# visionml/pytracking

Measured on AMD Instinct MI355X. Metric: frames/sec DiMP-50 online track (288x288, 5 SD iters), higher is better.
Workload: dtype f32; 1 GPU; BASELINE configs[1]: DiMP-50 single sequence per GPU; per frame classify(1x512x18x18) + arg-max + memory insert + DiMPSteepestDescentGN(5 it) over n=50x512x18x18, K=4; sequences_per_gpu=1, parallelism=1 independent sequences

## Files before the change

pytracking_amd/csrc/fast_passes.hip:

```cpp
#include "common.h"
#include "pt_internal.h"
#include "sd_common.h"
#include <type_traits>

#ifndef PT_ADJ_WAVES
#define PT_ADJ_WAVES 8
#endif
#ifndef PT_ADJ_UMAX
#define PT_ADJ_UMAX (128 / PT_ADJ_WAVES)
#endif
#ifndef PT_ADJ_UMAX_WIDE
#define PT_ADJ_UMAX_WIDE (192 / PT_ADJ_WAVES)
#endif
#ifndef PT_C2_CD
#define PT_C2_CD 2
#endif
#ifndef PT_C2_MINW
#define PT_C2_MINW 6
#endif
#ifndef PT_ADJ_PD
#define PT_ADJ_PD 3
#endif
#define PT_ADJ_AHEAD 5

#ifdef PT_STAMPS
static unsigned long long* g_pt_stamps = nullptr;
extern "C" void pt_debug_set_stamps(void* p) { g_pt_stamps = (unsigned long long*)p; }
#define PT_STAMP_ARG unsigned long long* stamps;
#define PT_STAMP_SET(a) (a).stamps = g_pt_stamps
#define PT_STAMP(a, k)                                                                                       \
    do {                                                                                                     \
        if ((a).stamps && (threadIdx.x & 63) == 0) {                                                         \
            unsigned long long* sp_ = (a).stamps + ((long)blockIdx.x * 16 + (threadIdx.x >> 6)) * 16;        \
            sp_[(k) < 8 ? (k) : (k) + 1] = (unsigned long long)wall_clock64();                               \
            if ((k) == 0) sp_[8] = (unsigned long long)__builtin_amdgcn_s_getreg((31 << 11) | 4) | (1ull << 32); \
        }                                                                                                    \
    } while (0)
#else
#define PT_STAMP_ARG
#define PT_STAMP_SET(a)
#define PT_STAMP(a, k)
#endif
#if defined(PT_STAMPS) && PT_STAMPS == 2
#define PT_STAMP_A(a, k)
#define PT_STAMP_A_ARRIVED(a, k, v)
#define PT_STAMP_B(a, k) PT_STAMP(a, k)
#else
#define PT_STAMP_A(a, k) PT_STAMP(a, k)
#ifdef PT_STAMPS
#define PT_STAMP_A_ARRIVED(a, k, v)                                                                          \
    do {                                                                                                     \
        asm volatile("" ::"v"(v));                                                                           \
        PT_STAMP(a, k);                                                                                      \
    } while (0)
#else
#define PT_STAMP_A_ARRIVED(a, k, v)
#endif
#define PT_STAMP_B(a, k)
#endif

PtFast pt_fast_plan(int n, int C, int H, int W, int KH, int KW, int OH, int OW) {
    PtFast p;
    p.ok = 0;
    p.n = n; p.C = C; p.H = H; p.W = W; p.KH = KH; p.KW = KW; p.OH = OH; p.OW = OW;
    p.HW = H * W; p.KK = KH * KW; p.OO = OH * OW;
    if ((p.HW % 4) != 0 || W < 4 || p.KK > 16) return p;
    if (C != 64 && C != 128 && C != 256 && C != 512 && C != 1024) return p;
    if ((long)n * p.HW >= (1L << 20)) return p;
    if ((long)n * C * p.HW * 4 >= (1L << 31)) return p;
    p.Q = p.HW / 4;
    p.TF = p.Q / 16;
    p.rem = p.Q % 16;
    p.left = (p.rem > 0 && p.rem <= 4) ? 1 : 0;
    p.tiles = p.TF + ((p.rem > 0 && !p.left) ? 1 : 0);
    if (p.TF < 1 || p.tiles > 16) return p;
    p.nh = 2 * p.tiles <= 10 ? 2 : 1;
    p.CX = C / 8;
    p.KSC = 8;
    if (C == 64) { p.CX = C; p.KSC = 1; }
    p.spw = 1;
    if (p.nh == 2 && p.KSC == 8 && p.CX / 4 <= 16 && (n % 2) == 0 && 8 * n > 256) { p.nh = 1; p.spw = 2; }
    p.NK = p.CX / 4 / p.nh;
    if (p.NK > 16) return p;
    p.mix = (p.spw == 2 && p.tiles == 5 && p.KK == 16 && p.NK >= 4) ? 1 : 0;
    p.HWp = 64 * (p.TF + (p.rem > 0 ? 1 : 0)) + 4;
    p.corr_threads = p.mix ? (2 * p.tiles + 2) * 64 : p.spw * p.nh * p.tiles * 64;
    p.corr_lds = ((size_t)p.CX * 16 + (size_t)p.spw * p.nh * p.KK * p.HWp) * sizeof(float);
    p.sa_direct = (KH == 4 && KW == 4 && p.CX * 16 >= 2 * W + 2) ? 1 : 0;
    if (p.sa_direct && p.HWp < p.HW + 2 * W + 2) p.corr_lds += (size_t)(p.HW + 2 * W + 2 - p.HWp) * sizeof(float);
    if (p.corr_lds > 150 * 1024) return p;
    p.CB = C / 16;
    p.bpx = p.CB / 8;
    p.NG = (int)(((long)n * p.HW + 15) / 16);
    p.KSPL = 0;
    p.E = p.OO <= 384 ? 6 : (p.OO <= 576 ? 9 : 16);
    const int umax = p.E == 9 ? PT_ADJ_UMAX_WIDE : PT_ADJ_UMAX;
    for (int ks = 8; ks <= (p.CB < 8 ? 64 : 16); ks *= 2) {
        const int gper = pt_ceil_div(p.NG, ks), U = pt_ceil_div(gper, PT_ADJ_WAVES);
        if (U <= umax) { p.gper = gper; p.U = U; p.KSPL = pt_ceil_div(p.NG, gper); break; }
    }
    if (p.KSPL == 0) return p;
    p.PH = H + KH - 1;
    p.PW = W + KW - 1;
    while ((p.PW % 16) != 8) ++p.PW;
    p.ns_max = (p.gper * 16 + p.HW - 1) / p.HW + 1;
    p.zn = (KH - 1) * p.PW + KW + 4;
    while (((p.ns_max * p.PH * p.PW + p.zn) % 4) != 0) ++p.zn;
    p.adj_lds = ((size_t)p.ns_max * p.PH * p.PW + p.zn + (size_t)5 * 4 * PT_ADJ_WAVES * umax) * sizeof(float);
    if (p.adj_lds > 96 * 1024 || p.OO > 1024) return p;
    if (H > 255 || W > 255 || n > 65535 || p.gper > 65535 || p.PH > 63 || p.PW > 63 || p.zn > 255 || p.ns_max > 63 || KH > 7 || KW > 7)
        return p;
    p.ok = 1;
    return p;
}

__device__ __forceinline__ int fdiv(int v, float inv_d) { return (int)(((float)v + 0.5f) * inv_d); }

struct Corr2Args {
    pt_gcf feat; long stride_n; pt_gcf filt; pt_gf spart;
    int n, C, H, W, KH, KW, OH, OW, CX, TF, rem, tiles, HWp, nh, KSC;
    int sa_direct;
    pt_gcf gpart; int KSPL; pt_gcf w; float reg; float step; pt_gf g_out; pt_gf anum_part;
    int slot; pt_gcf src; pt_gf copy_dst;
    PT_STAMP_ARG
};

__device__ __forceinline__ float corr2_filter_elem(const Corr2Args& a, int KK, int cx0, int e, bool publish, float& gsq) {
    const int cl = e >> 4, tp = e & 15;
    const bool ok = tp < KK;
    const long ge = (long)(cx0 + cl) * KK + (ok ? tp : 0);
    float v;
    if (a.gpart) {
        const long CKK = (long)a.C * KK;
        v = 0.f;
        for (int k = 0; k < a.KSPL; ++k) v += a.gpart[(long)k * CKK + ge];
        v += a.reg * a.w[ge];
        if (ok) {
            gsq += v * v;
            if (publish) a.g_out[ge] = v;
        }
    } else {
        v = a.filt[ge];
    }
    return ok ? v : 0.f;
}

template <int NK, bool LEFT, int FUSE, bool K16, int NH, bool MIX = false>
__global__ __launch_bounds__(1024, (NK <= 8 && NH == 2 ? PT_C2_MINW : 4)) void k_corr2(const float* h_feat, long h_stride, const float* h_filt, const float* h_w, const float* h_src, int h_slot,
                                                                              unsigned h_dims, unsigned h_geo, unsigned h_aux, Corr2Args a_arg) {
    extern __shared__ __attribute__((aligned(16))) float lds[];
    __shared__ float scratch[16];
    PT_STAMP(a_arg, 0);
    constexpr int EPT = 2;
    constexpr int FP = FUSE > 0 ? FUSE : 1;
    const int hC = (int)(h_dims >> 16), HW = (int)(h_dims & 0xffffu);
    const int h_tiles = (int)(h_geo & 31u), h_TF = (int)((h_geo >> 5) & 31u), h_rem = (int)((h_geo >> 10) & 15u);
    const int h_KSPL = (int)((h_geo >> 14) & 63u);
    const bool ksc16 = ((h_geo >> 20) & 1u) != 0, ksc1 = ((h_geo >> 21) & 1u) != 0, pair = ((h_geo >> 22) & 1u) != 0;
    const int wps = NH * h_tiles;
    const int nthreads = MIX ? (2 * h_tiles + 2) * 64 : (pair ? 2 : 1) * wps * 64;
    const int hCX = ksc1 ? hC : (ksc16 ? hC >> 4 : hC >> 3), hHWp = 64 * (h_TF + (h_rem > 0 ? 1 : 0)) + 4;
    const int b = blockIdx.x, xc = b & 7, q = b >> 3;
    const int x = ksc1 ? 0 : (ksc16 ? 2 * xc + (q & 1) : xc), i0 = ksc1 ? b : (ksc16 ? q >> 1 : q);
    const int KK = K16 ? 16 : a_arg.KH * a_arg.KW;
    const int lane = threadIdx.x & 63, wave = __builtin_amdgcn_readfirstlane(threadIdx.x >> 6);
    const int kq = lane >> 4, j = lane & 15;
    const bool half = MIX && wave < 4;
    const int ws = MIX ? (half ? wave >> 1 : (wave - 4 >= h_tiles - 1 ? 1 : 0)) : ((pair && wave >= wps) ? 1 : 0);
    const int wl = wave - ws * wps;
    const int i = pair ? 2 * i0 + ws : i0;
    const int h = MIX ? (half ? wave & 1 : 0) : (wl >= h_tiles ? 1 : 0);
    const int t = MIX ? (half ? 0 : wave - 3 - ws * (h_tiles - 1)) : wl - h * h_tiles;
    const bool lt = LEFT && t == 0 && (!MIX || h == 0);
    const int cx0 = hCX * x;
    const int nsl = hCX * 16;
    float* __restrict__ afilt = lds;
    float* __restrict__ Tl = lds + nsl + (long)(ws * NH + (MIX ? 0 : h)) * KK * hHWp;
    const bool over = h_src != nullptr && i == h_slot;
    const float* __restrict__ fi = over ? h_src : h_feat + (long)i * h_stride;
    const bool publish = FUSE != 0 && i0 == 0;
    const int h_n = (int)(h_geo >> 23);
    float lz_q = 0.f, lz_an = 0.f;

    constexpr bool k16 = K16;
    const int n4 = nsl >> 1;
    const int e4 = min((int)threadIdx.x, n4 - 1);
    f32x2 part4[FP], wv4 = {0, 0};
    float part[EPT][FP], wv[EPT];
    long gev[EPT];
    bool okv[EPT];
    if (k16) {
        const long g4 = ((long)cx0 * 16 >> 1) + e4;
        if (FUSE > 0) {
            const unsigned ckk_b = (unsigned)hC * 16u * 4u;
            const __amdgpu_buffer_rsrc_t rg = pt_rsrc(h_filt, (unsigned)h_KSPL * ckk_b);
#pragma unroll
            for (int k = 0; k < FP; ++k)
                part4[k] = __builtin_bit_cast(f32x2, __builtin_amdgcn_raw_buffer_load_b64(rg, (unsigned)g4 * 8u, (unsigned)min(k, h_KSPL - 1) * ckk_b, 0));
            wv4 = ((const f32x2*)h_w)[g4];
        } else if (FUSE < 0) {
            part4[0] = ((const f32x2*)h_filt)[g4];
            wv4 = ((const f32x2*)h_w)[g4];
            const float* __restrict__ anp = h_w + h_aux;
            lz_an = lane < (ksc16 ? 16 : (ksc1 ? 1 : 8)) ? anp[lane] : 0.f;
            lz_q = lane < h_n ? anp[64 + lane] : 0.f;
        } else {
            part4[0] = ((const f32x2*)h_filt)[g4];
        }
    } else {
#pragma unroll
        for (int q = 0; q < EPT; ++q) {
            const int e = threadIdx.x + q * nthreads;
            const int ec = min(e, nsl - 1);
            const int cl = ec >> 4, tp = ec & 15;
            okv[q] = e < nsl && tp < KK;
            gev[q] = (long)(cx0 + cl) * KK + (tp < KK ? tp : 0);
            if (FUSE > 0) {
                const long CKK = (long)hC * KK;
#pragma unroll
                for (int k = 0; k < FP; ++k) part[q][k] = h_filt[(long)min(k, h_KSPL - 1) * CKK + gev[q]];
                wv[q] = h_w[gev[q]];
            } else {
                part[q][0] = h_filt[gev[q]];
            }
        }
    }

    constexpr int CD = NK < PT_C2_CD ? NK : PT_C2_CD;
    const int cbase = cx0 + 4 * ((MIX ? 0 : h) * NK) + kq;
    const int pos = 64 * t + 4 * j + (half ? 2 * h : 0);
    const bool pv = pos < HW;
    const __amdgpu_buffer_rsrc_t fr = pt_rsrc(fi, (unsigned)hC * HW * 4u);
    const unsigned fo = ((unsigned)cbase * HW + (pv ? pos : 0)) * 4u;
    const int lpos = 64 * h_TF + j;
    const bool lv = lt && j < 4 * h_rem;
    const unsigned lo = lv ? ((unsigned)cbase * HW + lpos) * 4u : 0xFFFFFFF0u - 64u * (unsigned)HW * 4u;
    f32x4 bq[NK];
    float bl[NK];
    auto ldf = [&](int k) {
        if (MIX && half) {
            const f32x2 v = __builtin_bit_cast(f32x2, __builtin_amdgcn_raw_buffer_load_b64(fr, fo + (unsigned)(4 * k) * HW * 4u, 0, 0));
            bq[k] = (f32x4){v[0], v[1], 0.f, 0.f};
        } else {
            bq[k] = pt_bload4(fr, fo + (unsigned)(4 * k) * HW * 4u);
        }
    };
    auto ldq = [&](int k) {
        ldf(k);
        if (lt) bl[k] = pt_bload1(fr, lo + (unsigned)(4 * k) * HW * 4u);
    };
    if (lt) {
#pragma unroll
        for (int k = 0; k < CD; ++k) bl[k] = pt_bload1(fr, lo + (unsigned)(4 * k) * HW * 4u);
    }
#pragma unroll
    for (int k = 0; k < CD; ++k) ldf(k);
    __builtin_amdgcn_sched_barrier(0);
    const Corr2Args a = pt_late_args<Corr2Args>(56);
    PT_STAMP(a, 1);

    float gsq = 0.f;
    if (k16) {
        f32x2 v4;
        if (FUSE > 0) {
            v4 = (f32x2){0, 0};
#pragma unroll
            for (int k = 0; k < FP; ++k)
                if (k < h_KSPL) v4 += part4[k];
            v4 += a.reg * wv4;
            if ((int)threadIdx.x < n4) {
                gsq = v4[0] * v4[0] + v4[1] * v4[1];
                if (publish) ((f32x2*)a.g_out)[((long)cx0 * 16 >> 1) + e4] = v4;
            }
        } else if (FUSE < 0) {
            float qt = 0.f;
            for (int k = lane + 64; k < h_n; k += 64) qt += (h_w + h_aux)[64 + k];
            const float astep = sd_final_astep(lz_q, qt, lz_an, a.step, a.reg);
            v4 = (f32x2){sd_final_apply(part4[0][0], wv4[0], astep), sd_final_apply(part4[0][1], wv4[1], astep)};
            if ((int)threadIdx.x < n4 && publish) ((f32x2*)a.g_out)[((long)cx0 * 16 >> 1) + e4] = v4;
        } else {
            v4 = part4[0];
        }
        if ((int)threadIdx.x < n4) ((f32x2*)afilt)[e4] = v4;
        for (int q4 = threadIdx.x + nthreads; q4 < n4; q4 += nthreads)
            for (int m = 0; m < 2; ++m) afilt[2 * q4 + m] = corr2_filter_elem(a, KK, cx0, 2 * q4 + m, publish, gsq);
    } else {
#pragma unroll
        for (int q = 0; q < EPT; ++q) {
            const int e = threadIdx.x + q * nthreads;
            float v;
            if (FUSE > 0) {
                v = 0.f;
#pragma unroll
                for (int k = 0; k < FP; ++k) v += k < h_KSPL ? part[q][k] : 0.f;
                v += a.reg * wv[q];
                if (okv[q]) {
                    gsq += v * v;
                    if (publish) a.g_out[gev[q]] = v;
                }
            } else {
                v = part[q][0];
            }
            if (e < nsl) afilt[e] = okv[q] ? v : 0.f;
        }
        for (int e = threadIdx.x + EPT * nthreads; e < nsl; e += nthreads)
            afilt[e] = corr2_filter_elem(a, KK, cx0, e, publish, gsq);
    }
    if (FUSE > 0 && publish) {
        const float tot = block_sum(gsq, scratch, nthreads);
        if (threadIdx.x == 0) a.anum_part[x] = tot;
    }
    PT_STAMP(a, 2);
    __syncthreads();
    PT_STAMP(a, 3);

    auto mfma_phase = [&](auto half_c) {
        constexpr bool HALF = decltype(half_c)::value;
        f32x4 acc0 = {0, 0, 0, 0}, acc1 = {0, 0, 0, 0}, acc2 = {0, 0, 0, 0}, acc3 = {0, 0, 0, 0}, accL = {0, 0, 0, 0};
        float avv[NK];
#pragma unroll
        for (int k = 0; k < NK; ++k) avv[k] = afilt[(4 * ((MIX ? 0 : h) * NK + k) + kq) * 16 + j];
        __builtin_amdgcn_sched_barrier(0);
#pragma unroll
        for (int k = 0; k < NK; ++k) {
            if (k + CD < NK) ldq(k + CD);
            const float av = avv[k];
            acc0 = mfma16(av, bq[k][0], acc0);
            acc1 = mfma16(av, bq[k][1], acc1);
            if constexpr (!HALF) {
                acc2 = mfma16(av, bq[k][2], acc2);
                acc3 = mfma16(av, bq[k][3], acc3);
            }
            if (lt) accL = mfma16(av, bl[k], accL);
        }
        PT_STAMP(a, 4);
        if (over && a.copy_dst) {
            const pt_gf dp = a.copy_dst + pos + (long)cbase * HW;
            if (pv) {
#pragma unroll
                for (int k = 0; k < NK; ++k) {
                    if constexpr (HALF) *(f32x2*)(dp + (long)(4 * k) * HW) = (f32x2){bq[k][0], bq[k][1]};
                    else *(f32x4*)(dp + (long)(4 * k) * HW) = bq[k];
                }
            }
            if (lv) {
                const pt_gf dl = a.copy_dst + lpos + (long)cbase * HW;
#pragma unroll
                for (int k = 0; k < NK; ++k) dl[(long)(4 * k) * HW] = bl[k];
            }
        }

#pragma unroll
        for (int r = 0; r < 4; ++r) {
            const int row = 4 * kq + r;
            if (row < KK) {
                if constexpr (HALF) {
                    *(f32x2*)(Tl + row * hHWp + pos) = (f32x2){acc0[r], acc1[r]};
                } else {
                    f32x4 v = {acc0[r], acc1[r], acc2[r], acc3[r]};
                    *(f32x4*)(Tl + row * hHWp + pos) = v;
                }
                if (lt) Tl[row * hHWp + lpos] = accL[r];
            }
        }
    };
    if constexpr (MIX) {
        if (half) mfma_phase(std::true_type{});
        else mfma_phase(std::false_type{});
    } else {
        mfma_phase(std::false_type{});
    }
    PT_STAMP(a, 5);
    __syncthreads();
    PT_STAMP(a, 6);

    const int ph = a.KH / 2, pw = a.KW / 2, OO = a.OH * a.OW;
    const float inv_ow = 1.0f / (float)a.OW;
    const int nsm = pair ? 2 : 1;
    if (a.KH == 4 && a.KW == 4) {
      for (int s2 = 0; s2 < nsm; ++s2) {
        const float* __restrict__ T0 = lds + nsl + (long)s2 * NH * KK * hHWp;
        const float* __restrict__ T1 = T0 + (long)KK * hHWp;
        const pt_gf out = a.spart + ((long)x * a.n + (pair ? 2 * i0 + s2 : i0)) * OO;
        if (a.sa_direct) {
            const int su = 4 * hHWp + a.W, sv = hHWp + 1;
            for (int o = threadIdx.x; o < OO; o += nthreads) {
                const int y = fdiv(o, inv_ow), xx0 = o - y * a.OW;
                const int base = (y - 2) * a.W + (xx0 - 2);
                float t0[16], t1[16];
#pragma unroll
                for (int u = 0; u < 4; ++u)
#pragma unroll
                    for (int v = 0; v < 4; ++v) {
                        const int idx = base + (u * su + v * sv);
                        t0[u * 4 + v] = T0[idx];
                        if (NH == 2) t1[u * 4 + v] = T1[idx];
                    }
                int rok[4], cok[4];
#pragma unroll
                for (int u = 0; u < 4; ++u) rok[u] = (unsigned)(y + u - 2) < (unsigned)a.H ? -1 : 0;
#pragma unroll
                for (int v = 0; v < 4; ++v) cok[v] = (unsigned)(xx0 + v - 2) < (unsigned)a.W ? -1 : 0;
                __builtin_amdgcn_sched_barrier(0);
                float tv[16];
#pragma unroll
                for (int q = 0; q < 16; ++q) {
                    const float tsum = NH == 2 ? t0[q] + t1[q] : t0[q];
                    tv[q] = __builtin_bit_cast(float, __builtin_bit_cast(int, tsum) & (rok[q >> 2] & cok[q & 3]));
                }
                float s = 0.f;
#pragma unroll
                for (int q = 0; q < 16; ++q) s += tv[q];
                out[o] = s;
            }
            continue;
        }
        for (int o = threadIdx.x; o < OO; o += nthreads) {
            const int y = fdiv(o, inv_ow), xx0 = o - y * a.OW;
            float tv[16];
#pragma unroll
            for (int u = 0; u < 4; ++u) {
                const int yy = y + u - 2;
#pragma unroll
                for (int v = 0; v < 4; ++v) {
                    const int xx = xx0 + v - 2;
                    const bool ok = (unsigned)yy < (unsigned)a.H && (unsigned)xx < (unsigned)a.W;
                    const int idx = (u * 4 + v) * hHWp + (ok ? yy * a.W + xx : 0);
                    const float tsum = NH == 2 ? T0[idx] + T1[idx] : T0[idx];
                    tv[u * 4 + v] = ok ? tsum : 0.f;
                }
            }
            float s = 0.f;
#pragma unroll
            for (int q = 0; q < 16; ++q) s += tv[q];
            out[o] = s;
        }
      }
        PT_STAMP(a, 7);
        return;
    }
    for (int s2 = 0; s2 < nsm; ++s2) {
      const float* __restrict__ T0 = lds + nsl + (long)s2 * NH * KK * hHWp;
      const float* __restrict__ T1 = T0 + (long)KK * hHWp;
      const pt_gf out = a.spart + ((long)x * a.n + (pair ? 2 * i0 + s2 : i0)) * OO;
      for (int o = threadIdx.x; o < OO; o += nthreads) {
        const int y = fdiv(o, inv_ow), xx0 = o - y * a.OW;
        float s = 0.f;
        for (int u = 0; u < a.KH; ++u) {
            const int yy = y + u - ph;
            if ((unsigned)yy >= (unsigned)a.H) continue;
            for (int v = 0; v < a.KW; ++v) {
                const int xx = xx0 + v - pw;
                if ((unsigned)xx < (unsigned)a.W) {
                    const int idx = (u * a.KW + v) * hHWp + yy * a.W + xx;
                    s += NH == 2 ? T0[idx] + T1[idx] : T0[idx];
                }
            }
        }
        out[o] = s;
      }
    }
}

int pt_launch_corr2(const PtFast& p, const float* feat, long stride_n, const float* filt, float* spart, hipStream_t st,
                    const PtCorrFuse* fuse, int slot, const float* src, float* copy_dst, const PtCorrLazy* lazy) {
    Corr2Args a;
    a.feat = (pt_gcf)feat; a.stride_n = stride_n; a.filt = (pt_gcf)filt; a.spart = (pt_gf)spart;
    a.n = p.n; a.C = p.C; a.H = p.H; a.W = p.W; a.KH = p.KH; a.KW = p.KW; a.OH = p.OH; a.OW = p.OW;
    a.CX = p.CX; a.TF = p.TF; a.rem = p.rem; a.tiles = p.tiles; a.HWp = p.HWp; a.nh = p.nh; a.KSC = p.KSC;
    a.sa_direct = p.sa_direct;
    a.gpart = nullptr; a.KSPL = 0; a.w = nullptr; a.reg = 0.f; a.g_out = nullptr; a.anum_part = nullptr;
    if (fuse) {
        a.gpart = (pt_gcf)fuse->gpart; a.KSPL = fuse->KSPL; a.w = (pt_gcf)fuse->w; a.reg = fuse->reg; a.g_out = (pt_gf)fuse->g_out;
        a.anum_part = (pt_gf)fuse->anum_part;
    }
    a.slot = slot; a.src = (pt_gcf)src; a.copy_dst = (pt_gf)copy_dst;
    a.step = 0.f;
    unsigned h_aux = 0, h_nbits = 0;
    if (lazy) {
        if (fuse || p.KK != 16 || p.n > 511 || p.CX * 8 > p.corr_threads || !lazy->w_prev || !lazy->g || !lazy->anum || !lazy->w_out ||
            lazy->qs != lazy->anum + 64 || lazy->anum < lazy->g || (lazy->anum - lazy->g) > 0x3fffffffL)
            return PT_ERR_UNSUPPORTED;
        if (((uintptr_t)lazy->w_prev % 16) || ((uintptr_t)lazy->g % 16) || ((uintptr_t)lazy->w_out % 16)) return PT_ERR_UNSUPPORTED;
        a.filt = (pt_gcf)lazy->w_prev; a.w = (pt_gcf)lazy->g; a.g_out = (pt_gf)lazy->w_out; a.reg = lazy->reg_eps; a.step = lazy->step;
        h_aux = (unsigned)(lazy->anum - lazy->g);
        h_nbits = (unsigned)p.n << 23;
    }
    PT_STAMP_SET(a);
    if (((uintptr_t)feat % 16) || (stride_n % 4) || ((uintptr_t)src % 16) || ((uintptr_t)copy_dst % 16)) return PT_ERR_UNSUPPORTED;
    if ((long)p.n * stride_n * 4 >= (1L << 31)) return PT_ERR_UNSUPPORTED;
    if (p.KK == 16 && (((uintptr_t)filt % 16) || ((uintptr_t)a.gpart % 16) || ((uintptr_t)a.w % 16) || ((uintptr_t)a.g_out % 16)))
        return PT_ERR_UNSUPPORTED;
    dim3 grid(p.KSC * (p.n / p.spw)), block(p.corr_threads);
    if (p.C >= (1 << 16) || p.HW >= (1 << 16) || p.tiles > 31 || p.TF > 31 || p.rem > 15 || a.KSPL > 16) return PT_ERR_UNSUPPORTED;
    const unsigned h_dims = ((unsigned)p.C << 16) | (unsigned)p.HW;
    const unsigned h_geo = (unsigned)p.tiles | ((unsigned)p.TF << 5) | ((unsigned)p.rem << 10) | ((unsigned)a.KSPL << 14) |
                           ((p.KSC == 16 ? 1u : 0u) << 20) | ((p.KSC == 1 ? 1u : 0u) << 21) | ((p.spw == 2 ? 1u : 0u) << 22) | h_nbits;
#define PT_C2_HOT(FPTR) (const float*)a.feat, a.stride_n, (const float*)(FPTR), (const float*)a.w, (const float*)a.src, a.slot, h_dims, h_geo, h_aux
#define PT_C2G(NKV, LF, KF, NHV, MX)                                                                                  \
    do {                                                                                                         \
        if (lazy) { if constexpr (KF) hipLaunchKernelGGL((k_corr2<NKV, LF, -1, true, NHV, MX>), grid, block, p.corr_lds, st, PT_C2_HOT(a.filt), a); } \
        else if (!a.gpart) hipLaunchKernelGGL((k_corr2<NKV, LF, 0, KF, NHV, MX>), grid, block, p.corr_lds, st, PT_C2_HOT(a.filt), a);             \
        else if (pt_corr2_fuse_width(a.KSPL) == 8) hipLaunchKernelGGL((k_corr2<NKV, LF, 8, KF, NHV, MX>), grid, block, p.corr_lds, st, PT_C2_HOT(a.gpart), a);     \
        else hipLaunchKernelGGL((k_corr2<NKV, LF, 16, KF, NHV, MX>), grid, block, p.corr_lds, st, PT_C2_HOT(a.gpart), a);                     \
    } while (0)
#define PT_C2H(NKV, LF, KF)              \
    do {                                 \
        if (p.nh == 2) PT_C2G(NKV, LF, KF, 2, false); \
        else PT_C2G(NKV, LF, KF, 1, false);     \
    } while (0)
#define PT_C2F(NKV, LF)                  \
    do {                                 \
        if (p.KK == 16) PT_C2H(NKV, LF, true); \
        else PT_C2H(NKV, LF, false);     \
    } while (0)
#define PT_C2(NKV)                  \
    do {                            \
        if (p.left) PT_C2F(NKV, true); \
        else PT_C2F(NKV, false);    \
    } while (0)
#define PT_C2M(NKV)                                  \
    do {                                             \
        if (p.left) PT_C2G(NKV, true, true, 1, true);   \
        else PT_C2G(NKV, false, true, 1, true);      \
    } while (0)
    if (p.mix) {
        if (p.NK == 4) PT_C2M(4);
        else if (p.NK == 8) PT_C2M(8);
        else PT_C2M(16);
    }
    else if (p.NK == 2) PT_C2(2);
    else if (p.NK == 4) PT_C2(4);
    else if (p.NK == 8) PT_C2(8);
    else PT_C2(16);
#undef PT_C2_HOT
#undef PT_C2G
#undef PT_C2H
#undef PT_C2F
#undef PT_C2M
#undef PT_C2
    PT_CHECK_LAUNCH();
    return PT_OK;
}

struct Adj2Args {
    const float* feat; long stride_n; float* gpart;
    int n, C, H, W, KH, KW, OH, OW, NG, gper, U, bpx, PH, PW, ns_max, zn;
    const float* inp;
    SdArgs sd;
    int t, want_loss;
    PT_STAMP_ARG
};

struct Adj2SdLate {
    int n, CKK, has_sw, has_softmax_reg;
    float step, reg, alpha_eps, act_param, softmax_reg;
    int pad0;
    pt_gcf sw, s_in, w0;
    pt_gf mask, sws, s, sg, lms, g, lossp, w_iters;
};
struct Adj2Late {
    pt_gf gpart;
    int C, KH, KW, OH, OW, PH, PW, ns_max, zn, t, want_loss, pad1;
    Adj2SdLate sd;
    PT_STAMP_ARG
};
#ifndef PT_STAMPS
static_assert(sizeof(Adj2Late) == 46 * 4, "Adj2Late layout");
#endif

enum { V_PLAIN = 0, V_DIMP_RELU = 1, V_DIMP_BENT = 2, V_L2 = 3, V_PRDIMP = 4 };

template <int E>
struct PReg { f32x4 pk[E]; float s[E], sg[E], sw[E]; };

template <int V, int E>
__device__ __forceinline__ void sdp_load_hot(const float* __restrict__ pkp, int OO, int i, int lane, PReg<E>& r) {
    const long base = (long)i * OO;
#pragma unroll
    for (int e = 0; e < E; ++e) {
        const long q = base + min(lane + 64 * e, OO - 1);
        if (V == V_PLAIN) r.s[e] = pkp[q];
        else r.pk[e] = ((const f32x4*)pkp)[q];
    }
}
template <int V, int E, typename A>
__device__ __forceinline__ void sdp_load_rest(const A& a, int i, int lane, bool home, PReg<E>& r) {
    const int OO = a.OH * a.OW;
    const long base = (long)i * OO;
    const auto sgp = a.t > 0 ? pt_global((const float*)a.sd.sg) : pt_global((const float*)a.sd.s_in);
    if (V == V_DIMP_BENT) {
#pragma unroll
        for (int e = 0; e < E; ++e) r.sw[e] = pt_global((const float*)a.sd.sws)[base + min(lane + 64 * e, OO - 1)];
    }
    if (V != V_PLAIN && home) {
        const auto sin = pt_global((const float*)a.sd.s_in);
#pragma unroll
        for (int e = 0; e < E; ++e) {
            const long q = base + min(lane + 64 * e, OO - 1);
            r.s[e] = sin[q];
            r.sg[e] = sgp[q];
        }
    }
}
template <int V, int E, typename A>
__device__ __forceinline__ void sdp_load(const A& a, const float* __restrict__ pkp, int i, int lane, bool home, PReg<E>& r) {
    sdp_load_hot<V, E>(pkp, a.OH * a.OW, i, lane, r);
    sdp_load_rest<V, E>(a, i, lane, home, r);
}

struct Adj2InitLate {
    pt_gf label, cls_scores, cls_peak, cls_bb;
    const int* slot_dyn;
    int slot, mask_act;
    float feat_stride, bin_disp, gauss_sigma, hinge_thr;
};
static_assert(sizeof(Adj2InitLate) == 64, "Adj2InitLate: one 16-dword block");
#define PT_INIT_MAXKS 8
template <int E>
struct IReg { float sl[E][PT_INIT_MAXKS]; float bb[4]; };

template <int E>
__device__ __forceinline__ void sdi_load_hot(const float* __restrict__ spart, const float* __restrict__ bb, int n, int OO, int KS, int i, int lane,
                                             IReg<E>& r) {
    const unsigned stb = (unsigned)n * (unsigned)OO * 4u;
    const __amdgpu_buffer_rsrc_t rs = pt_rsrc(spart, (unsigned)KS * stb);
#pragma unroll
    for (int e = 0; e < E; ++e) {
        const unsigned vo = ((unsigned)i * (unsigned)OO + (unsigned)min(lane + 64 * e, OO - 1)) * 4u;
#pragma unroll
        for (int k = 0; k < PT_INIT_MAXKS; ++k)
            r.sl[e][k] = __builtin_bit_cast(float, __builtin_amdgcn_raw_buffer_load_b32(rs, vo, (unsigned)min(k, KS - 1) * stb, 0));
    }
#pragma unroll
    for (int k = 0; k < 4; ++k) r.bb[k] = bb[4 * i + k];
}

template <int V, int E, typename A>
__device__ __forceinline__ void sdi_make(const A& a, const Adj2InitLate& il, const float* __restrict__ lutl, int num_bins, int KS, int i, int lane,
                                         bool home, const IReg<E>& ir, PReg<E>& r) {
    const int OO = a.OH * a.OW;
    const long base = (long)i * OO;
    const float inv_ow = 1.0f / (float)a.OW;
    float s0[E];
#pragma unroll
    for (int e = 0; e < E; ++e) {
        float sm = 0.f;
#pragma unroll
        for (int k = 0; k < PT_INIT_MAXKS; ++k) sm += k < KS ? ir.sl[e][k] : 0.f;
        s0[e] = sm;
    }
    float b0 = ir.bb[0], b1 = ir.bb[1];
    const float b2 = ir.bb[2], b3 = ir.bb[3];
    const float off = (float)(a.KH % 2) * 0.5f;
    const int slot = il.slot_dyn ? *pt_global(il.slot_dyn) : il.slot;
    if (i == slot) {
        float best = -INFINITY;
        int besti = 0x7fffffff;
#pragma unroll
        for (int e = 0; e < E; ++e) {
            const int o = lane + 64 * e;
            if (o < OO && (s0[e] > best || (s0[e] == best && o < besti))) { best = s0[e]; besti = o; }
        }
#pragma unroll
        for (int sh = 32; sh > 0; sh >>= 1) {
            const float ov = __shfl_xor(best, sh, 64);
            const int oi = __shfl_xor(besti, sh, 64);
            if (ov > best || (ov == best && oi < besti)) { best = ov; besti = oi; }
        }
        const int row = besti / a.OW, col = besti - row * a.OW;
        b0 = ((float)col + off) * il.feat_stride - b2 * 0.5f;
        b1 = ((float)row + off) * il.feat_stride - b3 * 0.5f;
        if (home) {
// ... 457 lines not shown
```

Measured before the change: 9926 frames/s.

## Restructure corr2 feature prefetch pipeline around LDS barrier with specialized phases

Moves the feature-tile prefetch loads into the MFMA phase, issuing them just before a lighter LDS-only barrier instead of before the full __syncthreads. The prefetch depth becomes configurable with a default of 4, kept at 2 for the high-occupancy NH=2 variant. The phase is now specialized at compile time for half-width and left-tail waves, so register arrays are sized per variant and the runtime branches are removed. It also adds scalar readfirstlane hints and global-address-space pointer casts. Deeper prefetch raises VGPR pressure, which can lower occupancy, and the weaker barrier relies on global writes needing no ordering at that point.

```diff
diff --git a/pytracking_amd/csrc/fast_passes.hip b/pytracking_amd/csrc/fast_passes.hip
--- a/pytracking_amd/csrc/fast_passes.hip
+++ b/pytracking_amd/csrc/fast_passes.hip
@@ -12,8 +12,8 @@
 #ifndef PT_ADJ_UMAX_WIDE
 #define PT_ADJ_UMAX_WIDE (192 / PT_ADJ_WAVES)
 #endif
-#ifndef PT_C2_CD
-#define PT_C2_CD 2
+#ifndef PT_C2_D
+#define PT_C2_D 4
 #endif
 #ifndef PT_C2_MINW
 #define PT_C2_MINW 6
@@ -137,7 +137,7 @@
         v += a.reg * a.w[ge];
         if (ok) {
             gsq += v * v;
-            if (publish) a.g_out[ge] = v;
+            if (publish) pt_global(a.g_out)[ge] = v;
         }
     } else {
         v = a.filt[ge];
@@ -175,7 +175,7 @@
     const int cx0 = hCX * x;
     const int nsl = hCX * 16;
     float* __restrict__ afilt = lds;
-    float* __restrict__ Tl = lds + nsl + (long)(ws * NH + (MIX ? 0 : h)) * KK * hHWp;
+    float* __restrict__ Tl = lds + nsl + (long)__builtin_amdgcn_readfirstlane((ws * NH + (MIX ? 0 : h)) * KK * hHWp);
     const bool over = h_src != nullptr && i == h_slot;
     const float* __restrict__ fi = over ? h_src : h_feat + (long)i * h_stride;
     const bool publish = FUSE != 0 && i0 == 0;
@@ -194,9 +194,10 @@
         if (FUSE > 0) {
             const unsigned ckk_b = (unsigned)hC * 16u * 4u;
             const __amdgpu_buffer_rsrc_t rg = pt_rsrc(h_filt, (unsigned)h_KSPL * ckk_b);
+            const int klast = __builtin_amdgcn_readfirstlane(h_KSPL - 1);
 #pragma unroll
             for (int k = 0; k < FP; ++k)
-                part4[k] = __builtin_bit_cast(f32x2, __builtin_amdgcn_raw_buffer_load_b64(rg, (unsigned)g4 * 8u, (unsigned)min(k, h_KSPL - 1) * ckk_b, 0));
+                part4[k] = __builtin_bit_cast(f32x2, __builtin_amdgcn_raw_buffer_load_b64(rg, (unsigned)g4 * 8u, (unsigned)min(k, klast) * ckk_b, 0));
             wv4 = ((const f32x2*)h_w)[g4];
         } else if (FUSE < 0) {
             part4[0] = ((const f32x2*)h_filt)[g4];
@@ -226,7 +227,8 @@
         }
     }
 
-    constexpr int CD = NK < PT_C2_CD ? NK : PT_C2_CD;
+    constexpr int DW = (NK <= 8 && NH == 2 && PT_C2_D > 2) ? 2 : PT_C2_D;
+    constexpr int D = NK < DW ? NK : DW;
     const int cbase = cx0 + 4 * ((MIX ? 0 : h) * NK) + kq;
     const int pos = 64 * t + 4 * j + (half ? 2 * h : 0);
     const bool pv = pos < HW;
@@ -235,26 +237,6 @@
     const int lpos = 64 * h_TF + j;
     const bool lv = lt && j < 4 * h_rem;
     const unsigned lo = lv ? ((unsigned)cbase * HW + lpos) * 4u : 0xFFFFFFF0u - 64u * (unsigned)HW * 4u;
-    f32x4 bq[NK];
-    float bl[NK];
-    auto ldf = [&](int k) {
-        if (MIX && half) {
-            const f32x2 v = __builtin_bit_cast(f32x2, __builtin_amdgcn_raw_buffer_load_b64(fr, fo + (unsigned)(4 * k) * HW * 4u, 0, 0));
-            bq[k] = (f32x4){v[0], v[1], 0.f, 0.f};
-        } else {
-            bq[k] = pt_bload4(fr, fo + (unsigned)(4 * k) * HW * 4u);
-        }
-    };
-    auto ldq = [&](int k) {
-        ldf(k);
-        if (lt) bl[k] = pt_bload1(fr, lo + (unsigned)(4 * k) * HW * 4u);
-    };
-    if (lt) {
-#pragma unroll
-        for (int k = 0; k < CD; ++k) bl[k] = pt_bload1(fr, lo + (unsigned)(4 * k) * HW * 4u);
-    }
-#pragma unroll
-    for (int k = 0; k < CD; ++k) ldf(k);
     __builtin_amdgcn_sched_barrier(0);
     const Corr2Args a = pt_late_args<Corr2Args>(56);
     PT_STAMP(a, 1);
@@ -270,14 +252,14 @@
             v4 += a.reg * wv4;
             if ((int)threadIdx.x < n4) {
                 gsq = v4[0] * v4[0] + v4[1] * v4[1];
-                if (publish) ((f32x2*)a.g_out)[((long)cx0 * 16 >> 1) + e4] = v4;
+                if (publish) pt_global((f32x2*)a.g_out)[((long)cx0 * 16 >> 1) + e4] = v4;
             }
         } else if (FUSE < 0) {
             float qt = 0.f;
             for (int k = lane + 64; k < h_n; k += 64) qt += (h_w + h_aux)[64 + k];
             const float astep = sd_final_astep(lz_q, qt, lz_an, a.step, a.reg);
             v4 = (f32x2){sd_final_apply(part4[0][0], wv4[0], astep), sd_final_apply(part4[0][1], wv4[1], astep)};
-            if ((int)threadIdx.x < n4 && publish) ((f32x2*)a.g_out)[((long)cx0 * 16 >> 1) + e4] = v4;
+            if ((int)threadIdx.x < n4 && publish) pt_global((f32x2*)a.g_out)[((long)cx0 * 16 >> 1) + e4] = v4;
         } else {
             v4 = part4[0];
         }
@@ -296,7 +278,7 @@
                 v += a.reg * wv[q];
                 if (okv[q]) {
                     gsq += v * v;
-                    if (publish) a.g_out[gev[q]] = v;
+                    if (publish) pt_global(a.g_out)[gev[q]] = v;
                 }
             } else {
                 v = part[q][0];
@@ -308,14 +290,28 @@
     }
     if (FUSE > 0 && publish) {
         const float tot = block_sum(gsq, scratch, nthreads);
-        if (threadIdx.x == 0) a.anum_part[x] = tot;
-    }
-    PT_STAMP(a, 2);
-    __syncthreads();
-    PT_STAMP(a, 3);
-
-    auto mfma_phase = [&](auto half_c) {
+        if (threadIdx.x == 0) pt_global(a.anum_part)[x] = tot;
+    }
+    auto mfma_phase = [&](auto half_c, auto left_c) {
         constexpr bool HALF = decltype(half_c)::value;
+        constexpr bool LT = decltype(left_c)::value;
+        f32x4 bq[HALF ? 1 : NK];
+        f32x2 bh[HALF ? NK : 1];
+        float bl[LT ? NK : 1];
+        auto issue = [&](int k) {
+            const unsigned ko = (unsigned)(4 * k) * HW * 4u;
+            if constexpr (HALF) bh[k] = __builtin_bit_cast(f32x2, __builtin_amdgcn_raw_buffer_load_b64(fr, fo, ko, 0));
+            else bq[k] = __builtin_bit_cast(f32x4, __builtin_amdgcn_raw_buffer_load_b128(fr, fo, ko, 0));
+            if constexpr (LT) bl[k] = __builtin_bit_cast(float, __builtin_amdgcn_raw_buffer_load_b32(fr, lo, ko, 0));
+        };
+#pragma unroll
+        for (int k = 0; k < D; ++k) {
+            issue(k);
+            __builtin_amdgcn_sched_barrier(0);
+        }
+        PT_STAMP(a, 2);
+        pt_lds_barrier();
+        PT_STAMP(a, 3);
         f32x4 acc0 = {0, 0, 0, 0}, acc1 = {0, 0, 0, 0}, acc2 = {0, 0, 0, 0}, acc3 = {0, 0, 0, 0}, accL = {0, 0, 0, 0};
         float avv[NK];
 #pragma unroll
@@ -323,30 +319,39 @@
         __builtin_amdgcn_sched_barrier(0);
 #pragma unroll
         for (int k = 0; k < NK; ++k) {
-            if (k + CD < NK) ldq(k + CD);
+            if (k + D < NK) {
+                __builtin_amdgcn_sched_barrier(0);
+                issue(k + D);
+                __builtin_amdgcn_sched_barrier(0);
+            }
             const float av = avv[k];
-            acc0 = mfma16(av, bq[k][0], acc0);
-            acc1 = mfma16(av, bq[k][1], acc1);
-            if constexpr (!HALF) {
+            if constexpr (HALF) {
+                acc0 = mfma16(av, bh[k][0], acc0);
+                acc1 = mfma16(av, bh[k][1], acc1);
+            } else {
+                acc0 = mfma16(av, bq[k][0], acc0);
+                acc1 = mfma16(av, bq[k][1], acc1);
                 acc2 = mfma16(av, bq[k][2], acc2);
                 acc3 = mfma16(av, bq[k][3], acc3);
             }
-            if (lt) accL = mfma16(av, bl[k], accL);
+            if constexpr (LT) accL = mfma16(av, bl[k], accL);
         }
         PT_STAMP(a, 4);
         if (over && a.copy_dst) {
-            const pt_gf dp = a.copy_dst + pos + (long)cbase * HW;
+            const pt_gptr<float> dp = pt_global(a.copy_dst) + (fo >> 2);
             if (pv) {
 #pragma unroll
                 for (int k = 0; k < NK; ++k) {
-                    if constexpr (HALF) *(f32x2*)(dp + (long)(4 * k) * HW) = (f32x2){bq[k][0], bq[k][1]};
-                    else *(f32x4*)(dp + (long)(4 * k) * HW) = bq[k];
+                    if constexpr (HALF) *(pt_gptr<f32x2>)(dp + (long)(4 * k) * HW) = bh[k];
+                    else *(pt_gptr<f32x4>)(dp + (long)(4 * k) * HW) = bq[k];
                 }
             }
-            if (lv) {
-                const pt_gf dl = a.copy_dst + lpos + (long)cbase * HW;
-#pragma unroll
-                for (int k = 0; k < NK; ++k) dl[(long)(4 * k) * HW] = bl[k];
+            if constexpr (LT) {
+                if (lv) {
+                    const pt_gptr<float> dl = pt_global(a.copy_dst) + (lo >> 2);
+#pragma unroll
+                    for (int k = 0; k < NK; ++k) dl[(long)(4 * k) * HW] = bl[k];
+                }
             }
         }
 
@@ -360,15 +365,21 @@
                     f32x4 v = {acc0[r], acc1[r], acc2[r], acc3[r]};
                     *(f32x4*)(Tl + row * hHWp + pos) = v;
                 }
-                if (lt) Tl[row * hHWp + lpos] = accL[r];
+                if constexpr (LT) Tl[row * hHWp + lpos] = accL[r];
             }
         }
     };
+    constexpr std::true_type yes{};
+    constexpr std::false_type no{};
     if constexpr (MIX) {
-        if (half) mfma_phase(std::true_type{});
-        else mfma_phase(std::false_type{});
+        if (half && lt) mfma_phase(yes, std::integral_constant<bool, LEFT>{});
+        else if (half) mfma_phase(yes, no);
+        else mfma_phase(no, no);
+    } else if constexpr (LEFT) {
+        if (lt) mfma_phase(no, yes);
+        else mfma_phase(no, no);
     } else {
-        mfma_phase(std::false_type{});
+        mfma_phase(no, no);
     }
     PT_STAMP(a, 5);
     __syncthreads();
```

After: 10100 frames/s, median of 6. 1.8% higher.
